# LowLevelAI/GLARE

Hardware: AMD Instinct MI355X
Metric: enhanced images/sec (400x600) (higher is better)
Workload: dtype fp16; 1 GPU; LOL eval15-shaped 400x600 inference, batch=8 per GPU, full encoder->flow->VQ->decoder->AFT (BASELINE configs[1]); batch_per_gpu=8, global_batch=8, input=3x400x600 (reflect-padded to 420x620), parallelism=dp1, streams_per_gpu=2, exchange=none (1 GPU), ranks_seen=1, weights=random, name-seeded (no checkpoints offline)

## Files before the change

glare_amd/csrc/conv_igemm.hip:

```cpp
#include "conv_igemm_kernel.h"

namespace {

__device__ __forceinline__ void pack_weight_chunk(const float* __restrict__ w, a16_t* __restrict__ out, long long chunk, int Cout, int Cin,
                                                  int KS, int TN, int KSTEPS, int n_stages, int dgrad, int Cin_real) {
  long long t = chunk;
  const int n = t % TN; t /= TN;
  const int khalf = t % 2; t /= 2;
  const int ks = t % KSTEPS; t /= KSTEPS;
  const int KK = KS * KS;
  const int tap = t % KK; t /= KK;
  const int s = t % n_stages; t /= n_stages;
  const int ct = (int)t;
  const int co = ct * TN + n;
  const int ci0 = (s * KSTEPS + ks) * 16 + khalf * 8;
  float v[8];
#pragma unroll
  for (int e = 0; e < 8; ++e) {
    const int ci = ci0 + e;
    v[e] = 0.f;
    if (dgrad) {
      if (co < Cout && ci < Cin_real) v[e] = w[((size_t)ci * Cout + co) * KK + (KK - 1 - tap)];
    } else if (co < Cout && ci < Cin) {
      v[e] = w[((size_t)co * Cin + ci) * KK + tap];
// ... 253 lines not shown
}

extern "C" int glare_conv2d_bf16(const glare_conv_desc* d, glare_stream_t stream_) {
  if (!d || !d->in || !d->weight_packed || !d->out) return GLARE_ERR_INVALID;
  if (d->B <= 0 || d->H <= 0 || d->W <= 0 || d->Cin <= 0 || d->Cout <= 0) return GLARE_ERR_INVALID;
  if (d->ksize != 1 && d->ksize != 3) return GLARE_ERR_UNSUPPORTED;
  if (d->stride != 1 && d->stride != 2) return GLARE_ERR_UNSUPPORTED;
  if (d->stride == 2 && (d->ksize != 3 || d->upsample)) return GLARE_ERR_UNSUPPORTED;
  const bool subpix = d->upsample == 2;
  if (subpix && (d->ksize != 3 || d->stride != 1)) return GLARE_ERR_UNSUPPORTED;
  if ((d->Cin % 8) || (d->in_pitch % 8) || (d->in_off % 8)) return GLARE_ERR_UNSUPPORTED;
  if (d->in2 && ((d->Cin2 % 8) || (d->in2_pitch % 8) || (d->in2_off % 8) || d->Cin2 <= 0)) return GLARE_ERR_UNSUPPORTED;
  if (d->out_mode < GLARE_OUT_NHWC_BF16 || d->out_mode > GLARE_OUT_PLANAR_BF16) return GLARE_ERR_INVALID;
  if (d->residual && d->out_mode > GLARE_OUT_NHWC_F32) return GLARE_ERR_UNSUPPORTED;
  if (d->in_off + d->Cin > d->in_pitch || d->out_off + d->Cout > d->out_pitch) return GLARE_ERR_INVALID;

  ConvParams p;
  p.in0 = (const a16_t*)d->in;
  p.in1 = (const a16_t*)d->in2;
  p.wpk = (const a16_t*)d->weight_packed;
  p.bias = d->bias;
  p.res = (const a16_t*)d->residual;
  p.out = d->out;
  p.B = d->B; p.H = d->H; p.W = d->W;
  p.IHs = (d->upsample && !subpix) ? 2 * d->H : d->H;
  p.IWs = (d->upsample && !subpix) ? 2 * d->W : d->W;
  if (d->stride == 2) {
    p.OH = (p.IHs + 1 - 3) / 2 + 1;
    p.OW = (p.IWs + 1 - 3) / 2 + 1;
  } else {
    p.OH = p.IHs; p.OW = p.IWs;
  }
  if (d->k_wrap < 0 || d->k_wrap > 2 || (d->k_wrap == 2 && !(d->in2 && d->Cin2 == d->Cin))) return GLARE_ERR_INVALID;
  if (d->k_wrap == 2 && (d->ksize != 3 || d->gn_coef || d->upsample || d->Cin % 16)) return GLARE_ERR_UNSUPPORTED;
  p.k_wrap = d->k_wrap;
  p.Cin0 = d->Cin; p.Cin1 = d->in2 ? d->Cin2 : 0; p.CinTot = p.Cin0 + p.Cin1 + (p.k_wrap ? p.Cin0 : 0);
  p.p0 = d->in_pitch; p.o0 = d->in_off; p.p1 = d->in2_pitch; p.o1 = d->in2_off;
  p.Cout = d->Cout; p.opitch = d->out_pitch; p.ooff = d->out_off;
  p.rpitch = d->res_pitch; p.roff = d->res_off;
  p.upsample = subpix ? 0 : d->upsample; p.act = d->act; p.out_mode = d->out_mode;
  p.plane_pitch = d->plane_pitch > 0 ? d->plane_pitch : (long long)p.OH * p.OW;
  if (p.plane_pitch < (long long)p.OH * p.OW) return GLARE_ERR_INVALID;
  if (d->cout_tile != 0 && (d->upsample == 2 || (d->cout_tile != 32 && d->cout_tile != 64 && d->cout_tile != 128))) return GLARE_ERR_INVALID;
  const Variant v = pick_variant(d->ksize, d->Cout, d->cout_tile);
  if (d->gn_partial && v.tn == 32 && d->Cout > 32) return GLARE_ERR_UNSUPPORTED;
  const int kc = 16 * v.ksteps;
  if ((p.in1 || p.k_wrap) && (p.Cin0 % kc)) return GLARE_ERR_UNSUPPORTED;
  if (p.k_wrap && (p.Cin1 % kc)) return GLARE_ERR_UNSUPPORTED;
  if (p.k_wrap && (subpix || d->upsample)) return GLARE_ERR_UNSUPPORTED;
  p.n_stages = (p.CinTot + kc - 1) / kc;
  {
    const long long b0 = (long long)p.H * p.W * p.p0 * 2, b1 = p.in1 ? (long long)p.H * p.W * p.p1 * 2 : 0;
    if (b0 >= 0x7ff00000LL || b1 >= 0x7ff00000LL) return GLARE_ERR_UNSUPPORTED;
    p.in0_bytes = (unsigned)b0;
    p.in1_bytes = (unsigned)b1;
    const long long br = d->residual ? (long long)p.OH * p.OW * p.rpitch * 2 : 0;
    p.res_bytes = (br > 0 && br < 0x7ff00000LL && !subpix) ? (unsigned)br : 0u;
    static const bool no_prefetch = getenv("GLARE_CONV_NO_RES_PREFETCH") != nullptr;
    if (no_prefetch) p.res_bytes = 0;
  }
  p.tiles_x = cdiv(p.OW, TW); p.tiles_y = 0; p.co_tiles = cdiv(p.Cout, v.tn);
  p.n_blocks = 0;
  p.gn_part = d->gn_partial;
  p.gn_nparts = 0;
  p.res_lo = (const a16_t*)d->residual_lo;
  p.out_lo = (a16_t*)d->out_lo;
  p.groups = d->groups > 1 ? d->groups : 1;
  p.g_in_step = d->group_in_step; p.g_out_step = d->group_out_step; p.g_bias_step = d->Cout; p.g_w_elems = 0;
  if (p.groups > 1) {
    if ((d->in2 && !(p.k_wrap && d->in2_pitch == d->in_pitch && d->Cin2 == d->Cin)) || d->residual || d->gn_partial || subpix || p.groups > 65535)
      return GLARE_ERR_UNSUPPORTED;
    if ((d->group_in_step % 8) || d->in_off + (long long)(p.groups - 1) * d->group_in_step + d->Cin > d->in_pitch ||
        d->out_off + (long long)(p.groups - 1) * d->group_out_step + d->Cout > d->out_pitch || d->group_out_step < 0 || d->group_in_step < 0)
      return GLARE_ERR_INVALID;
    p.g_w_elems = glare_conv2d_packed_weight_elems_tile(d->Cout, p.CinTot, d->ksize, d->cout_tile);
    if (d->in2 && d->in2_off + (long long)(p.groups - 1) * d->group_in_step + d->Cin2 > d->in2_pitch) return GLARE_ERR_INVALID;
  }
  p.gn_coef = d->gn_coef; p.gn_swish = d->gn_swish;
  if (p.gn_coef && (d->ksize != 3 || d->stride != 1 || d->in2 || p.k_wrap || d->upsample || p.groups > 1 || p.out_lo || d->in_off != 0 ||
                    d->Cin > 512))
    return GLARE_ERR_UNSUPPORTED;
  if (p.res_lo && !(p.res && p.out_lo)) return GLARE_ERR_INVALID;
  p.fast_epilogue = (d->out_mode == GLARE_OUT_NHWC_BF16) && !(p.Cout % 8) && !(p.opitch % 8) && !(p.ooff % 8) &&
                    (!p.res || (!(p.rpitch % 8) && !(p.roff % 8)));
  hipStream_t stream = (hipStream_t)stream_;

  if (p.out_lo) {
    if (subpix || d->upsample || !p.fast_epilogue) return GLARE_ERR_UNSUPPORTED;
    if (d->ksize == 1) return glare_conv_launch_k1(p, v.tn, true, stream);
    return d->stride == 2 ? glare_conv_launch_k3s2(p, v.tn, true, stream) : glare_conv_launch_k3s1(p, v.tn, true, stream);
  }
  if (subpix) {
    if (!p.fast_epilogue) return GLARE_ERR_UNSUPPORTED;
    return glare_conv_launch_k2(p, v.tn, stream);
  }
  if (d->ksize == 1) return glare_conv_launch_k1(p, v.tn, false, stream);
  if (d->stride == 2) return glare_conv_launch_k3s2(p, v.tn, false, stream);
  return glare_conv_launch_k3s1(p, v.tn, false, stream);
}

extern "C" long long glare_conv2d_gn_partial_elems(int B, int OH, int OW, int Cout) {
  if (B <= 0 || OH <= 0 || OW <= 0 || Cout <= 0) return GLARE_ERR_INVALID;
  const long long parts = (long long)cdiv(OW, TW) * cdiv(OH, 8) * 2;
  return (long long)B * parts * (Cout / 4) * 2;
}

extern "C" long long glare_conv2d_upsample_gn_partial_elems(int B, int H, int W, int Cout) {
  if (B <= 0 || H <= 0 || W <= 0 || Cout <= 0) return GLARE_ERR_INVALID;
  return 4 * glare_conv2d_gn_partial_elems(B, H, W, Cout);
}

extern "C" int glare_conv2d_upsample_gn_reduce(const float* gn_partial, float* stats_out, int B, int H, int W, int Cout,
                                               glare_stream_t stream) {
// ... 14 lines not shown
```

glare_amd/csrc/conv_igemm_k3s1.hip:

```cpp
#include "conv_igemm_kernel.h"

int glare_conv_launch_k3s1(const ConvParams& p, int tn, bool hilo, hipStream_t stream) {
  if (hilo) return tn == 128 ? launch<3, 1, 4, 2, 2, 2, 1, true>(p, stream) : GLARE_ERR_UNSUPPORTED;
  const int epi = conv_pick_epilogue(p, true);
  if (p.gn_coef) return (tn == 128 && epi == EPI_FAST) ? launch<3, 1, 4, 2, 2, 2, 1, false, true>(p, stream) : GLARE_ERR_UNSUPPORTED;
  if (epi == EPI_PLANAR) return glare_conv_launch_k3s1_planar(p, tn, stream);
  if (epi == EPI_GENERAL) return glare_conv_launch_k3s1_general(p, tn, stream);
  if (tn == 128) return launch<3, 1, 4, 2, 2, 2, 1>(p, stream);
  if (tn == 64) return launch<3, 1, 4, 1, 2, 2, 1>(p, stream);
  return launch<3, 1, 2, 1, 4, 1, 1>(p, stream);
}
```

glare_amd/csrc/conv_igemm_kernel.h:

```cpp
#pragma once
#include <type_traits>

#include "common.h"



struct ConvParams {
  const a16_t* in0;
  const a16_t* in1;
  const a16_t* wpk;
  const float* bias;
  const a16_t* res;
  void* out;
  int B, H, W;
  int IHs, IWs;
  int OH, OW;
  int Cin0, Cin1, CinTot;
  int p0, o0, p1, o1;
  int Cout, opitch, ooff, rpitch, roff;
  int upsample, act, out_mode;
  long long plane_pitch;
  int tiles_x, tiles_y, co_tiles, n_blocks, n_stages;
  int fast_epilogue;
  unsigned in0_bytes, in1_bytes;
  unsigned res_bytes;
  float* gn_part;
  int gn_nparts;
  const a16_t* res_lo;
  a16_t* out_lo;
  int groups, g_in_step, g_out_step, g_bias_step;
  long long g_w_elems;
  int k_wrap;
  const float* gn_coef;
  int gn_swish;
};

enum { EPI_FAST = 0,
       EPI_PLANAR = 1,
       EPI_GENERAL = 2 };
__host__ inline int conv_pick_epilogue(const ConvParams& p, bool planar_kernel) {
  const bool expk = p.act == GLARE_ACT_SIGMOID || p.act == GLARE_ACT_SWISH;
  if (p.out_mode == GLARE_OUT_NHWC_BF16 && p.fast_epilogue && !(p.res == nullptr && expk)) return EPI_FAST;
  if (planar_kernel && p.out_mode == GLARE_OUT_PLANAR_F32 && !p.res && !expk) return EPI_PLANAR;
  return EPI_GENERAL;
}

int glare_conv_launch_k3s1(const ConvParams& p, int tn, bool hilo, hipStream_t stream);
int glare_conv_launch_k3s1_planar(const ConvParams& p, int tn, hipStream_t stream);
int glare_conv_launch_k3s1_general(const ConvParams& p, int tn, hipStream_t stream);
int glare_conv_launch_k3s2(const ConvParams& p, int tn, bool hilo, hipStream_t stream);
int glare_conv_launch_k3s2_general(const ConvParams& p, int tn, hipStream_t stream);
int glare_conv_launch_k1(const ConvParams& p, int tn, bool hilo, hipStream_t stream);
int glare_conv_launch_k1_general(const ConvParams& p, int tn, hipStream_t stream);
int glare_conv_launch_k2(const ConvParams& p, int tn, hipStream_t stream);

namespace {

constexpr int TW = 32;



template <int KS, int STRIDE, int TH>
struct TileGeom {
  static constexpr int IH = (TH - 1) * STRIDE + KS;
  static constexpr int IW = (TW - 1) * STRIDE + KS;
  static constexpr int NPOS = IH * IW;
  static constexpr int PAD = (KS == 3 && STRIDE == 1) ? 1 : 0;
};

template <int N, typename F>
__device__ __forceinline__ void static_for(F&& f) {
  if constexpr (N > 0) {
    static_for<N - 1>(f);
    f(std::integral_constant<int, N - 1>{});
  }
}



__device__ __forceinline__ int fresh_lane_id() {
  int l;
  asm volatile("v_mbcnt_lo_u32_b32 %0, -1, 0\n\tv_mbcnt_hi_u32_b32 %0, -1, %0" : "=v"(l));
  return l;
}

__device__ __forceinline__ void gn_prologue_piece(u32x4* slot, const float* cf, int swish) {
  __builtin_amdgcn_sched_barrier(0);
  u32x4 v = *slot;
#pragma unroll
  for (int e = 0; e < 4; ++e) {
    const f32x4 q = *reinterpret_cast<const f32x4*>(cf + 4 * e);
    float lo = alo(v[e]) * q[0] + q[1];
    float hi = ahi(v[e]) * q[2] + q[3];
    if (swish) { lo = swishf_(lo); hi = swishf_(hi); }
    v[e] = pack_a2(lo, hi);
    __builtin_amdgcn_sched_barrier(0);
  }
  *slot = v;
  __builtin_amdgcn_sched_barrier(0);
}

template <int KS, int STRIDE, int MT, int NT, int WM, int WN, int KSTEPS, bool HILO = false, bool GNP = false, int EPI = EPI_FAST>
__global__ __launch_bounds__(64 * WM * WN, ((STRIDE == 1 && WM * WN == 4) ? 3 : 2)) void conv_igemm_kernel(const ConvParams p_in) {
  ConvParams p = p_in;
  if (p.groups > 1) {
    const int g = blockIdx.y;
    p.o0 += g * p.g_in_step;
    p.o1 += g * p.g_in_step;
    p.ooff += g * p.g_out_step;
    p.wpk += (size_t)g * p.g_w_elems;
    if (p.bias) p.bias += g * p.g_bias_step;
  }
  constexpr int TH = WM * MT;
  constexpr int NW = WM * WN;
  using G = TileGeom<KS, STRIDE, TH>;
  static_assert(NW == 4 || NW == 6 || NW == 8, "wave layout");
  constexpr int TN = WN * NT * 32;
  constexpr int A_CHUNKS = KSTEPS * 2 * G::NPOS;
  constexpr int A_INSTR = (A_CHUNKS + 63) / 64;
  constexpr int A_SLOTS = A_INSTR * 64;
  constexpr int A_PER_W = (A_INSTR + NW - 1) / NW;
  constexpr int B_CHUNKS = KS * KSTEPS * 2 * TN;
  static_assert(B_CHUNKS % 64 == 0, "B stage is a whole number of wave DMAs");
  constexpr int B_INSTR = B_CHUNKS / 64;
  constexpr int B_PER_W = (B_INSTR + NW - 1) / NW;
  constexpr int KC = 16 * KSTEPS;

  extern __shared__ __attribute__((aligned(16))) char smem[];
  u32x4* lA = reinterpret_cast<u32x4*>(smem);
  u32x4* lB = lA + 2 * A_SLOTS;

  int bid = blockIdx.x;
// ... 23 lines not shown
#pragma unroll
    for (int j = 0; j < NT; ++j)
#pragma unroll
      for (int r = 0; r < 16; ++r) acc[i][j][r] = 0.f;

  constexpr unsigned A_OOB = 0x80000000u;
  unsigned a_vo0[A_PER_W], a_vo1[A_PER_W];
  int a_ck[A_PER_W];
#pragma unroll
  for (int i = 0; i < A_PER_W; ++i) {
    const int c = (wave + NW * i) * 64 + lane;
    a_vo0[i] = a_vo1[i] = A_OOB;
    a_ck[i] = 0;
    if (c < A_CHUNKS) {
      const int prow = c / (2 * KSTEPS * G::IW), rem = c % (2 * KSTEPS * G::IW);
      const int kk = rem / G::IW, pos = prow * G::IW + rem % G::IW;
      a_ck[i] = kk * 8;
      const int iy = iy0 + pos / G::IW, ix = ix0 + pos % G::IW;
      if (iy >= 0 && iy < p.IHs && ix >= 0 && ix < p.IWs) {
        const int sy = p.upsample ? (iy >> 1) : iy, sx = p.upsample ? (ix >> 1) : ix;
        const unsigned pix = (unsigned)(sy * p.W + sx);
        a_vo0[i] = (pix * (unsigned)p.p0 + (unsigned)(p.o0 + kk * 8)) * 2u;
        if constexpr (!GNP) a_vo1[i] = (pix * (unsigned)p.p1 + (unsigned)(p.o1 + kk * 8)) * 2u;
      }
    }
  }
  const size_t img = (size_t)b * p.H * p.W;
  const __amdgpu_buffer_rsrc_t arsrc0 =
      __builtin_amdgcn_make_buffer_rsrc(const_cast<a16_t*>(p.in0 + img * p.p0), 0, (int)p.in0_bytes, 0x00020000);
  const __amdgpu_buffer_rsrc_t arsrc1 = __builtin_amdgcn_make_buffer_rsrc(
      const_cast<a16_t*>(p.in1 ? p.in1 + img * p.p1 : p.in0), 0, (int)(p.in1 ? p.in1_bytes : p.in0_bytes), 0x00020000);
  const a16_t* wbase = p.wpk + ((size_t)phase * p.co_tiles + ct) * p.n_stages * (size_t)(KS * B_CHUNKS) * 8;

  const bool reuse = KS == 3 && !GNP && p.k_wrap == 2;
  const int n_pair = reuse ? 2 * (p.Cin0 / KC) : 0;
  auto a_is_new = [&](int stage) { return !(reuse && stage < n_pair && (stage & 1)); };
  auto issue_a = [&](int chunk, int buf, int i_lo = 0, int i_hi = 1 << 20) {
    const int c0 = chunk * KC;
    bool src0 = GNP || c0 < p.Cin0 || c0 >= p.Cin0 + p.Cin1;
    int cbase = c0 < p.Cin0 ? c0 : (src0 ? c0 - p.Cin0 - p.Cin1 : c0 - p.Cin0);
    if (reuse) {
      src0 = chunk < n_pair;
      cbase = src0 ? (chunk >> 1) * KC : (chunk - n_pair) * KC;
    }
    const int climit = src0 ? p.Cin0 : p.Cin1;
#pragma unroll
    for (int i = 0; i < A_PER_W; ++i) {
      const int j = wave + NW * i;
      if (i >= i_lo && i < i_hi && j < A_INSTR) {
        unsigned vo = src0 ? a_vo0[i] : a_vo1[i];
        if (cbase + a_ck[i] >= climit) vo = A_OOB;
        if (src0)
          __builtin_amdgcn_raw_ptr_buffer_load_lds(arsrc0, (__attribute__((address_space(3))) void*)(lA + buf * A_SLOTS + j * 64), 16, vo,
                                                   cbase * 2, 0, 0);
        else
          __builtin_amdgcn_raw_ptr_buffer_load_lds(arsrc1, (__attribute__((address_space(3))) void*)(lA + buf * A_SLOTS + j * 64), 16, vo,
                                                   cbase * 2, 0, 0);
      }
    }
  };
  const __amdgpu_buffer_rsrc_t wrsrc = __builtin_amdgcn_make_buffer_rsrc(
      const_cast<a16_t*>(wbase), 0, (int)((size_t)p.n_stages * KS * B_CHUNKS * 16), 0x00020000);
  const int lane16 = lane * 16;
  auto issue_b = [&](int bstage, int buf, int i_lo = 0, int i_hi = 1 << 20) {
#pragma unroll
    for (int i = 0; i < B_PER_W; ++i) {
      const int j = wave + NW * i;
      if (i >= i_lo && i < i_hi && j < B_INSTR)
        __builtin_amdgcn_raw_ptr_buffer_load_lds(wrsrc, (__attribute__((address_space(3))) void*)(lB + buf * B_CHUNKS + j * 64),
                                                 16, lane16, (bstage * B_CHUNKS + j * 64) * 16, 0, 0);
    }
  };

  [[maybe_unused]] auto prefetch_residual = [&](int free_buf) {
    if constexpr (KS == 3 && STRIDE == 1 && NW == 4 && TN == 128) {
      static_assert(A_SLOTS * 16 >= NW * 4 * 256, "room for the prefetch's landing zone");
      const size_t rimg = (size_t)b * p.OH * p.OW * p.rpitch;
#pragma unroll
      for (int k = 0; k < 2; ++k) {
        const int l = (wave * 2 + k) * 64 + lane;
        const int oy = oy0 + (l >> 6), ox = ox0 + ((l >> 1) & 31), co = ct * TN + (l & 1) * 64;
        const unsigned vo = (oy < p.OH && ox < p.OW && co < p.Cout)
                                ? (unsigned)(((oy * p.OW + ox) * p.rpitch + p.roff + co) * 2) : 0x80000000u;
        const __amdgpu_buffer_rsrc_t rr = __builtin_amdgcn_make_buffer_rsrc(const_cast<a16_t*>(p.res + rimg), 0, (int)p.res_bytes, 0x00020000);
        __builtin_amdgcn_raw_ptr_buffer_load_lds(rr, (__attribute__((address_space(3))) void*)(lA + free_buf * A_SLOTS + (wave * 4 + k) * 16),
                                                 4, vo, 0, 0, 0);
        if constexpr (HILO) {
          if (p.res_lo) {
            const __amdgpu_buffer_rsrc_t rl =
                __builtin_amdgcn_make_buffer_rsrc(const_cast<a16_t*>(p.res_lo + rimg), 0, (int)p.res_bytes, 0x00020000);
            __builtin_amdgcn_raw_ptr_buffer_load_lds(rl, (__attribute__((address_space(3))) void*)(lA + free_buf * A_SLOTS + (wave * 4 + 2 + k) * 16),
                                                     4, vo, 0, 0, 0);
          }
        }
      }
    }
  };

  [[maybe_unused]] float* lC = reinterpret_cast<float*>(lB + 2 * B_CHUNKS);
  [[maybe_unused]] auto gn_transform = [&](int chunk, int buf) {
    if constexpr (GNP) {
      const int c0 = chunk * KC;
#pragma unroll
      for (int i = 0; i < A_PER_W; ++i) {
        const int j = wave + NW * i;
        if (j < A_INSTR && a_vo0[i] != A_OOB && c0 + a_ck[i] < p.Cin0) {
          int ln = fresh_lane_id(), ck = a_ck[i];
          asm volatile("" : "+v"(ln), "+v"(ck));
          gn_prologue_piece(lA + buf * A_SLOTS + j * 64 + ln, lC + (c0 + ck) * 2, p.gn_swish);
        }
      }
    }
  };
  if constexpr (GNP) {
    const float* src = p.gn_coef + (size_t)b * p.Cin0 * 2;
    for (int i = tid; i < p.Cin0 * 2; i += 64 * NW) lC[i] = src[i];
    __syncthreads();
  }

  const int khalf = lane >> 5, px = lane & 31;
  const int n_bstages = p.n_stages * KS;
  issue_a(0, 0);
  issue_b(0, 0);
  int bs = 0;
  int a_cnt = 0;
  for (int chunk = 0; chunk < p.n_stages; ++chunk) {
    const u32x4* cA = lA + (a_cnt & 1) * A_SLOTS;
    const bool next_new = chunk + 1 < p.n_stages && a_is_new(chunk + 1);
#pragma unroll
    for (int trow = 0; trow < KS; ++trow, ++bs) {
      asm volatile("s_waitcnt vmcnt(0)" ::: "memory");
      if constexpr (GNP) {
        if (trow == 0 && chunk == 0) gn_transform(0, 0);
        if (trow == 1 && chunk + 1 < p.n_stages) gn_transform(chunk + 1, (a_cnt + 1) & 1);
      }
      __syncthreads();
      constexpr int NGRP = KS * KSTEPS;
      [[maybe_unused]] constexpr int B_PG = (B_PER_W + NGRP - 1) / NGRP, A_PG = (A_PER_W + NGRP - 1) / NGRP;
      const bool more_b = bs + 1 < n_bstages, more_a = trow == 0 && next_new;
      if (trow == 0 && chunk + 1 == p.n_stages && p.res_bytes) prefetch_residual((a_cnt + 1) & 1);
      const u32x4* cB = lB + (bs & 1) * B_CHUNKS;
#pragma unroll
      for (int tcol = 0; tcol < KS; ++tcol) {
#pragma unroll
        for (int ks = 0; ks < KSTEPS; ++ks) {
          {
            const int grp = tcol * KSTEPS + ks;
            if (more_b) issue_b(bs + 1, (bs + 1) & 1, grp * B_PG, (grp + 1) * B_PG);
            if (more_a) issue_a(chunk + 1, (a_cnt + 1) & 1, grp * A_PG, (grp + 1) * A_PG);
          }
          a16x8 bf[NT], af[MT];
#pragma unroll
          for (int j = 0; j < NT; ++j) {
            const int co = (wn * NT + j) * 32 + px;
            bf[j] = __builtin_bit_cast(a16x8, cB[((tcol * KSTEPS + ks) * 2 + khalf) * TN + co]);
          }
#pragma unroll
          for (int i = 0; i < MT; ++i) {
            const int row = wm * MT + i;
            af[i] = __builtin_bit_cast(a16x8, cA[((row * STRIDE + trow) * (2 * KSTEPS) + ks * 2 + khalf) * G::IW + px * STRIDE + tcol]);
          }
#pragma unroll
          for (int i = 0; i < MT; ++i)
#pragma unroll
            for (int j = 0; j < NT; ++j)
              acc[i][j] = mfma_a16_32x32x16(af[i], bf[j], acc[i][j], 0, 0, 0);
        }
      }
    }
    if (next_new) ++a_cnt;
  }

  if constexpr (HILO) {
    constexpr int ROWF = NT * 128 + 16;
    constexpr int CPR = NT * 4;
    static_assert(NW * 32 * ROWF <= (2 * A_SLOTS + 2 * B_CHUNKS) * 16, "hi/lo epilogue slab fits the pipeline LDS");
    static_assert(KS != 2, "the sub-pixel form has no hi/lo epilogue");
    __syncthreads();
    char* slab = smem + wave * (32 * ROWF);
    const int lane = fresh_lane_id();
    const int ncol = lane & 31, rhalf = lane >> 5;
    float gs0 = 0.f, gq0 = 0.f, gs1 = 0.f, gq1 = 0.f;
// ... 287 lines not shown
        } else {
          if (co_ok && row_ok) {
            const size_t base = ((size_t)b * p.opitch + p.ooff + co) * (size_t)p.plane_pitch + (size_t)oy * p.OW + xb;
#pragma unroll
            for (int e = 0; e < 4; ++e) {
              if (xb + e < p.OW) {
                const float y = act_any(v[e], asel);
                if (p.out_mode == GLARE_OUT_PLANAR_F32)
                  reinterpret_cast<float*>(p.out)[base + e] = y;
                else
                  reinterpret_cast<a16_t*>(p.out)[base + e] = f2a(y);
              }
            }
          }
        }
      }
    });
  });
  }
}

template <int KS, int STRIDE, int MT, int NT, int WM, int WN, int KSTEPS, bool HILO = false, bool GNP = false, int EPI = EPI_FAST>
int launch(const ConvParams& p_in, hipStream_t stream) {
  using G = TileGeom<KS, STRIDE, WM * MT>;
  constexpr int TN = WN * NT * 32;
  ConvParams p = p_in;
  p.tiles_y = cdiv(p.OH, WM * MT);
  const long long nb = (long long)p.B * p.tiles_x * p.tiles_y * p.co_tiles * (KS == 2 ? 4 : 1);
  if (nb > 0x7fffffffLL) return GLARE_ERR_INVALID;
  p.n_blocks = (int)nb;
  p.gn_nparts = p.tiles_x * cdiv(p.OH, 8) * 2 * (KS == 2 ? 4 : 1);
  if (p.gn_part && !(p.fast_epilogue && p.Cout % 32 == 0)) return GLARE_ERR_UNSUPPORTED;
  if (p.gn_part && !HILO && EPI != EPI_FAST) return GLARE_ERR_UNSUPPORTED;
  const size_t lds = (size_t)(2 * (((KSTEPS * 2 * G::NPOS + 63) / 64) * 64) + 2 * KS * KSTEPS * 2 * TN) * 16 + (GNP ? (size_t)p.Cin0 * 8 : 0);
  constexpr bool PLANAR_KERNEL = !HILO && KS == 3 && STRIDE == 1 && WM * WN == 4;
  if (!HILO && conv_pick_epilogue(p, PLANAR_KERNEL) != EPI) return GLARE_ERR_INVALID;
  auto kern = conv_igemm_kernel<KS, STRIDE, MT, NT, WM, WN, KSTEPS, HILO, GNP, EPI>;
  if (lds > 64 * 1024 &&
      hipFuncSetAttribute((const void*)kern, hipFuncAttributeMaxDynamicSharedMemorySize, (int)lds) != hipSuccess)
    return GLARE_ERR_LAUNCH;
  hipLaunchKernelGGL(kern, dim3(p.n_blocks, p.groups > 1 ? p.groups : 1), dim3(64 * WM * WN), lds, stream, p);
  return glare_launch_status();
}

}
```

glare_amd/modules/encoder_decoder.py:

```python
import math
import os
import threading

import torch
import torch.nn as nn

from .. import autograd as A
from .. import ops
from ._base import HipModule, packed_conv, to_nchw, to_nhwc


GN_FUSED = True


def Normalize(in_channels):
    return nn.GroupNorm(num_groups=32, num_channels=in_channels, eps=1e-6, affine=True)


def gn_swish(x, norm, swish=True, pair=False):
    return ops.groupnorm(x, norm.weight.detach().float(), norm.bias.detach().float(), swish=swish, eps=norm.eps, pair=pair)


def is_hilo(x):
    return getattr(x, "_lo", None) is not None
# ... 4 lines not shown


def conv_t(x, conv, **kw):
    return A.conv2d(x, conv.weight, conv.bias, **kw)


HILO_STREAM = os.environ.get("GLARE_HILO_STREAM", "1") != "0"
FP32_CLASS = os.environ.get("GLARE_FP32_CLASS", "1") != "0"


_FP32_TLS = threading.local()


def fp32_class_on():
    v = getattr(_FP32_TLS, "value", None)
    return FP32_CLASS if v is None else v


class fp32_class:

    def __init__(self, on):
        self.on = bool(on)

    def __enter__(self):
        self._prev = getattr(_FP32_TLS, "value", None)
        _FP32_TLS.value = self.on
        return self

    def __exit__(self, *exc):
        _FP32_TLS.value = self._prev


GN_PROLOGUE = os.environ.get("GLARE_GN_PROLOGUE", "0") == "1"
SUBPIXEL_UPSAMPLE = True
FOLD_PROJ_INTO_V = True
SHARED_KV_ATTENTION = True
GN_FOLDED_ATTENTION = True


class Upsample(HipModule):
    def __init__(self, in_channels, with_conv=True):
        super().__init__()
        assert with_conv, "GLARE always resamples with a conv (resamp_with_conv=True)"
        self.with_conv = with_conv
        self.conv = nn.Conv2d(in_channels, in_channels, 3, 1, 1)

    def forward_nhwc(self, x, **kw):
        if SUBPIXEL_UPSAMPLE:
            pc = self._packed(("conv_subpixel", id(self.conv)),
                              lambda: ops.PackedConv(self.conv.weight, self.conv.bias, upsample_subpixel=True))
        else:
            pc = packed_conv(self, self.conv)
        return ops.conv2d(x, pc, upsample=True, gn_stats=GN_FUSED and self.conv.out_channels % 128 == 0, **kw)

    def train_nhwc(self, x):
        return conv_t(x, self.conv, upsample=True)

    def forward(self, x):
        return to_nchw(self.forward_nhwc(to_nhwc(x)))


class Downsample(HipModule):
    def __init__(self, in_channels, with_conv=True):
        super().__init__()
        assert with_conv
        self.with_conv = with_conv
        self.conv = nn.Conv2d(in_channels, in_channels, 3, 2, 0)

    def forward_nhwc(self, x, split=0):
        return ops.conv2d(x, packed_conv(self, self.conv, split=split), stride=2,
                          gn_stats=GN_FUSED and self.conv.out_channels % 128 == 0, hilo=is_hilo(x))

    def train_nhwc(self, x):
        return conv_t(x, self.conv, stride=2)

    def forward(self, x):
        return to_nchw(self.forward_nhwc(to_nhwc(x)))


class ResnetBlock(HipModule):
    def __init__(self, *, in_channels, out_channels=None, conv_shortcut=False, dropout=0.0, temb_channels=0):
        super().__init__()
        assert temb_channels == 0 and not conv_shortcut and dropout == 0.0
        out_channels = in_channels if out_channels is None else out_channels
        self.in_channels, self.out_channels = in_channels, out_channels
        self.norm1 = Normalize(in_channels)
        self.conv1 = nn.Conv2d(in_channels, out_channels, 3, 1, 1)
        self.norm2 = Normalize(out_channels)
        self.conv2 = nn.Conv2d(out_channels, out_channels, 3, 1, 1)
        if in_channels != out_channels:
            self.nin_shortcut = nn.Conv2d(in_channels, out_channels, 1, 1, 0)

    def forward_nhwc(self, x, out=None, out_off=0, split=0):
        fuse = GN_FUSED and self.out_channels % 128 == 0
        hl = is_hilo(x)
        if split:
            assert hl and out is None and split == 3
            h = ops.conv2d(gn_swish(x, self.norm1, pair=True), packed_conv(self, self.conv1, split=3), gn_stats=fuse, hilo=True)
            h = gn_swish(h, self.norm2, pair=True)
            res = x if self.in_channels == self.out_channels else ops.conv2d(x, packed_conv(self, self.nin_shortcut, split=3), hilo=True)
            return ops.conv2d(h, packed_conv(self, self.conv2, split=3), residual=res, gn_stats=fuse, hilo=True)
        if GN_PROLOGUE and not hl and self.in_channels <= 128 and getattr(x, "_gn_stats", None) is not None:
            coef = lambda t, n: ops.groupnorm_coeffs(t, n.weight.detach().float(), n.bias.detach().float(), n.eps)
            h = ops.conv2d(x, packed_conv(self, self.conv1), gn_stats=fuse, gn_prologue=(coef(x, self.norm1), True))
            if fuse and self.out_channels <= 128 and out is None:
                return ops.conv2d(h, packed_conv(self, self.conv2), gn_prologue=(coef(h, self.norm2), True),
                                  residual=x if self.in_channels == self.out_channels else ops.conv2d(x, packed_conv(self, self.nin_shortcut)),
                                  gn_stats=fuse)
        else:
            h = ops.conv2d(gn_swish(x, self.norm1), packed_conv(self, self.conv1), gn_stats=fuse)
        h = gn_swish(h, self.norm2)
        res = x if self.in_channels == self.out_channels else ops.conv2d(x, packed_conv(self, self.nin_shortcut), hilo=hl)
        return ops.conv2d(h, packed_conv(self, self.conv2), residual=res, out=out, out_off=out_off,
                          gn_stats=fuse and out is None, hilo=hl)

    def train_nhwc(self, x):
        x, xr = A.fork(x)
        h = conv_t(gn_swish_t(x, self.norm1), self.conv1)
        h = gn_swish_t(h, self.norm2)
        res = xr if self.in_channels == self.out_channels else conv_t(xr, self.nin_shortcut)
        return conv_t(h, self.conv2, residual=res)

    def forward(self, x, temb=None):
        return to_nchw(self.forward_nhwc(to_nhwc(x)))


class AttnBlock(HipModule):
    def __init__(self, in_channels):
        super().__init__()
        assert in_channels % 32 == 0, "AttnBlock: channels must be a multiple of 32 (GroupNorm(32), 32-wide GEMM k-steps)"
        self.in_channels = in_channels
        self.norm = Normalize(in_channels)
        self.q = nn.Conv2d(in_channels, in_channels, 1)
        self.k = nn.Conv2d(in_channels, in_channels, 1)
# ... 265 lines not shown
```

glare_amd/ops.py:

```python
import ctypes
import os

import torch

from . import _lib
from ._lib import act_dtype, check, host_f32, inference_precision, precision, ptr, require_cuda, stream_handle, use_precision


def vq_nearest(z_tokens, codebook, want_zq=True):
    require_cuda(z_tokens, codebook)
    assert z_tokens.dtype == torch.float32 and codebook.dtype == torch.float32
    z_tokens = z_tokens.contiguous()
    codebook = codebook.contiguous()
    n, dim = z_tokens.shape
    idx = torch.empty(n, dtype=torch.int64, device=z_tokens.device)
    zq = torch.empty_like(z_tokens) if want_zq else None
    check(_lib.lib().glare_vq_nearest_f32(ptr(z_tokens), ptr(codebook), n, codebook.shape[0], dim, ptr(idx), ptr(zq),
                                          stream_handle()), "glare_vq_nearest_f32")
    return idx, zq


_K = _lib.constants()
ACT = {name: _K["GLARE_ACT_" + name.upper()] for name in ("none", "relu", "sigmoid", "swish")}
OUT_NHWC_BF16, OUT_NHWC_F32, OUT_PLANAR_F32, OUT_PLANAR_BF16 = (_K["GLARE_OUT_" + n] for n in ("NHWC_BF16", "NHWC_F32", "PLANAR_F32", "PLANAR_BF16"))
# ... 424 lines not shown
def _ws_eligible(pc, x, cin, in_off, x2, stride, upsample, out_mode, out, out_off, residual, res_off, gn_stats, hilo, gn_prologue):
    if not (CONV1X1_WEIGHT_STATIONARY and x2 is None and stride == 1 and not upsample and out_mode == OUT_NHWC_BF16 and cin == pc.cin
            and x.shape[3] % 8 == 0 and in_off % 8 == 0
            and (out is None or (out.dtype == act_dtype() and out.shape[3] % 8 == 0 and out_off % 8 == 0))
            and (residual is None or (residual.shape[3] % 8 == 0 and res_off % 8 == 0))):
        return False
    whole = out is None or (out_off == 0 and out.shape[3] == pc.cout)
    if pc.split == 0:
        return pc.w16 is not None and (not gn_stats or out is None)
    if pc.split == 3:
        return (pc.ksize == 1 and pc.w16_lo is not None and gn_prologue is None and (not hilo or whole)
                and (not gn_stats or (pc.cout % 128 == 0 and whole)))
    return False


def conv2d(x, pc, *, x2=None, cin=None, in_off=0, cin2=None, in2_off=0, stride=1, upsample=False, act="none",
           residual=None, res_off=0, out=None, out_off=0, out_mode=OUT_NHWC_BF16, plane_pitch=0, gn_stats=False, hilo=False,
           gn_prologue=None):
    require_cuda(x, x2, residual, out)
    assert x.dtype == act_dtype() and x.dim() == 4 and x.is_contiguous(), (x.dtype, act_dtype())
    assert pc.packed.dtype == x.dtype, "filter packed under another precision"
    B, H, W, pitch = x.shape
    cin = pitch - in_off if cin is None else cin
    split = pc.split
    _count_conv_flops(pc, B * H * W * (4 if upsample else 1) // (stride * stride))
    if hilo and pc.ksize == 1 and not split:
        assert x2 is None and stride == 1 and not upsample and out is None and cin == pc.cin and pc.w16 is not None
        return _conv1x1_ws(x, pc, cin, in_off, act, residual, res_off, None, 0, gn_stats, True)
    if _ws_eligible(pc, x, cin, in_off, x2, stride, upsample, out_mode, out, out_off, residual, res_off, gn_stats, hilo, gn_prologue):
        return _conv1x1_ws(x, pc, cin, in_off, act, residual, res_off, out, out_off, gn_stats, hilo)
    cin2_total = 0
    if split:
        assert x2 is None and not upsample and cin == pc.cin, (cin, pc.cin)
        assert pc.k_wrap != 2 or gn_prologue is None
    elif x2 is not None:
        assert x2.dtype == act_dtype() and x2.is_contiguous() and x2.shape[:3] == x.shape[:3]
        cin2_total = x2.shape[3] - in2_off if cin2 is None else cin2
    assert pc.cin == cin + cin2_total, (pc.cin, cin, cin2_total)
    IH, IW = (2 * H, 2 * W) if upsample else (H, W)
    OH, OW = ((IH + 1 - 3) // 2 + 1, (IW + 1 - 3) // 2 + 1) if stride == 2 else (IH, IW)
    if out is None:
        if out_mode in (OUT_NHWC_BF16, OUT_NHWC_F32):
            out = torch.empty(B, OH, OW, pc.cout, dtype=act_dtype() if out_mode == OUT_NHWC_BF16 else torch.float32, device=x.device)
        else:
            pp = plane_pitch or OH * OW
            dt = torch.float32 if out_mode == OUT_PLANAR_F32 else act_dtype()
            out = torch.empty(B, pc.cout, pp, dtype=dt, device=x.device)
            if pp > OH * OW:
                out[:, :, OH * OW:].zero_()
    assert out.is_contiguous()
    if (AUTO_COUT_TILE and pc.ksize == 3 and pc.cout > 64 and pc.cout_tile == 0 and not pc.subpixel and pc._src is not None
            and not hilo and gn_prologue is None):
        tile = conv_cout_tile(B, OH, OW, pc.cout)
        if tile == 32 and gn_stats:
            tile = 64
        if tile:
            if tile not in pc._tiles:
                pc._tiles[tile] = PackedConv(pc._src[0], pc._src[1], dgrad_pad=pc._src[2], cout_tile=tile)
            pc = pc._tiles[tile]
    d = _conv_desc(x, pc, cin, in_off)
    if x2 is not None:
        d.in2, d.Cin2, d.in2_pitch, d.in2_off = x2.data_ptr(), cin2_total, x2.shape[3], in2_off
    if out_mode in (OUT_NHWC_BF16, OUT_NHWC_F32):
        d.out_pitch = out.shape[3]
    else:
        d.out_pitch, d.plane_pitch = out.shape[1], out.shape[2]
    d.out, d.out_off = out.data_ptr(), out_off
    if residual is not None:
        assert residual.dtype == act_dtype() and residual.is_contiguous()
        d.residual, d.res_pitch, d.res_off = residual.data_ptr(), residual.shape[3], res_off
    out_lo = None
    if hilo:
        assert out_mode == OUT_NHWC_BF16 and out_off == 0 and out.shape[3] == pc.cout
        out_lo = getattr(out, "_lo", None)
        if out_lo is None:
            out_lo = torch.empty_like(out)
        d.out_lo = out_lo.data_ptr()
        rlo = getattr(residual, "_lo", None) if residual is not None else None
        if rlo is not None:
            assert rlo.shape == residual.shape and rlo.dtype == residual.dtype and rlo.is_contiguous()
            d.residual_lo = rlo.data_ptr()
    if gn_prologue is not None:
        coef, swish = gn_prologue
        assert coef.dtype == torch.float32 and coef.is_contiguous() and tuple(coef.shape) == (B, cin, 2)
        assert pc.ksize == 3 and stride == 1 and x2 is None and not upsample and not split and not hilo and in_off == 0
        d.gn_coef, d.gn_swish = coef.data_ptr(), int(bool(swish))
    assert not pc.subpixel or upsample, "a sub-pixel packed filter only implements the upsample conv"
    d.stride, d.upsample, d.act, d.out_mode = stride, (2 if pc.subpixel else int(bool(upsample))), ACT[act], out_mode
    lib = _lib.lib()
    gn = None
    if gn_stats:
        assert out_mode == OUT_NHWC_BF16 and pc.cout % 128 == 0 and out_off == 0 and out.shape[3] == pc.cout
        gn = _GnStats("glare_conv2d_upsample", (B, H, W, pc.cout), x.device) if pc.subpixel else _GnStats("glare_conv2d", (B, OH, OW, pc.cout), x.device)
        d.gn_partial = gn.partial.data_ptr()
    if LAUNCH_EVENTS is not None and pc.ksize == 3:
        opix = B * OH * OW
        esz = 2 if out_mode in (OUT_NHWC_BF16, OUT_PLANAR_BF16) else 4
        with _timed_launch("conv3x3_split" if split else "conv3x3", 2.0 * opix * 9 * pc.cin * pc.cout,
                           2.0 * B * H * W * pc.cin * (2 if split == 3 else 1) + esz * opix * pc.cout * (2 if hilo else 1)
                           + 2.0 * 9 * pc.cin * pc.cout * (split or 1)):
            check(lib.glare_conv2d_bf16(ctypes.byref(d), stream_handle()), "glare_conv2d_bf16")
    else:
        check(lib.glare_conv2d_bf16(ctypes.byref(d), stream_handle()), "glare_conv2d_bf16")
    if gn is not None:
        gn.reduce(out)
    if out_lo is not None:
        out._lo = out_lo
    return out


def _workspace(nbytes, device):
    return torch.empty(max(int(nbytes), 16), dtype=torch.uint8, device=device)


def conv2d_smallcin(x, strides, shape_bhw, weight, bias=None, act="none", out=None, out_off=0, out_f32=False, hilo=False):
    require_cuda(x, weight, bias, out)
    B, H, W = shape_bhw
    w = weight.detach().float().contiguous()
# ... 476 lines not shown
```

Before: 63.57 images/sec.

## Fuse hi/lo pair GroupNorm+swish prologue into split-3 conv for 128-channel resblocks

Adds a GN-prologue variant of the hi/lo (split=3, k_wrap) 3x3 conv kernel. It loads both the hi and lo halves of each input tile, sums them, applies the GroupNorm affine plus swish in LDS, and re-splits into hi/lo before the MMA. This replaces the separate gn_swish pass that wrote a normalized pair tensor. It is enabled for 128-channel resblocks in split mode. The cost is extra LDS space for a companion buffer, additional loads, and more complex scheduling inside the main loop.

```diff
diff --git a/glare_amd/csrc/conv_igemm.hip b/glare_amd/csrc/conv_igemm.hip
--- a/glare_amd/csrc/conv_igemm.hip
+++ b/glare_amd/csrc/conv_igemm.hip
@@ -309,7 +309,7 @@
     p.OH = p.IHs; p.OW = p.IWs;
   }
   if (d->k_wrap < 0 || d->k_wrap > 2 || (d->k_wrap == 2 && !(d->in2 && d->Cin2 == d->Cin))) return GLARE_ERR_INVALID;
-  if (d->k_wrap == 2 && (d->ksize != 3 || d->gn_coef || d->upsample || d->Cin % 16)) return GLARE_ERR_UNSUPPORTED;
+  if (d->k_wrap == 2 && (d->ksize != 3 || d->upsample || d->Cin % 16)) return GLARE_ERR_UNSUPPORTED;
   p.k_wrap = d->k_wrap;
   p.Cin0 = d->Cin; p.Cin1 = d->in2 ? d->Cin2 : 0; p.CinTot = p.Cin0 + p.Cin1 + (p.k_wrap ? p.Cin0 : 0);
   p.p0 = d->in_pitch; p.o0 = d->in_off; p.p1 = d->in2_pitch; p.o1 = d->in2_off;
@@ -354,8 +354,10 @@
     if (d->in2 && d->in2_off + (long long)(p.groups - 1) * d->group_in_step + d->Cin2 > d->in2_pitch) return GLARE_ERR_INVALID;
   }
   p.gn_coef = d->gn_coef; p.gn_swish = d->gn_swish;
-  if (p.gn_coef && (d->ksize != 3 || d->stride != 1 || d->in2 || p.k_wrap || d->upsample || p.groups > 1 || p.out_lo || d->in_off != 0 ||
-                    d->Cin > 512))
+  if (p.gn_coef && (d->ksize != 3 || d->stride != 1 || d->upsample || p.groups > 1 || d->in_off != 0 || d->Cin > 512))
+    return GLARE_ERR_UNSUPPORTED;
+  if (p.gn_coef && (p.k_wrap || d->in2 || p.out_lo) &&
+      !(p.k_wrap && d->in2 && p.out_lo && d->Cin2 == d->Cin && d->in2_pitch == d->in_pitch && d->in2_off == 0 && d->Cin % 16 == 0))
     return GLARE_ERR_UNSUPPORTED;
   if (p.res_lo && !(p.res && p.out_lo)) return GLARE_ERR_INVALID;
   p.fast_epilogue = (d->out_mode == GLARE_OUT_NHWC_BF16) && !(p.Cout % 8) && !(p.opitch % 8) && !(p.ooff % 8) &&
diff --git a/glare_amd/csrc/conv_igemm_k3s1.hip b/glare_amd/csrc/conv_igemm_k3s1.hip
--- a/glare_amd/csrc/conv_igemm_k3s1.hip
+++ b/glare_amd/csrc/conv_igemm_k3s1.hip
@@ -1,6 +1,7 @@
 #include "conv_igemm_kernel.h"
 
 int glare_conv_launch_k3s1(const ConvParams& p, int tn, bool hilo, hipStream_t stream) {
+  if (hilo && p.gn_coef) return glare_conv_launch_k3s1_gnpair(p, tn, stream);
   if (hilo) return tn == 128 ? launch<3, 1, 4, 2, 2, 2, 1, true>(p, stream) : GLARE_ERR_UNSUPPORTED;
   const int epi = conv_pick_epilogue(p, true);
   if (p.gn_coef) return (tn == 128 && epi == EPI_FAST) ? launch<3, 1, 4, 2, 2, 2, 1, false, true>(p, stream) : GLARE_ERR_UNSUPPORTED;
diff --git a/glare_amd/csrc/conv_igemm_k3s1_gnpair.hip b/glare_amd/csrc/conv_igemm_k3s1_gnpair.hip
--- /dev/null
+++ b/glare_amd/csrc/conv_igemm_k3s1_gnpair.hip
@@ -0,0 +1,6 @@
+#include "conv_igemm_kernel.h"
+
+int glare_conv_launch_k3s1_gnpair(const ConvParams& p, int tn, hipStream_t stream) {
+  if (tn != 128 || !p.gn_coef || !p.k_wrap || !p.in1 || !p.out_lo) return GLARE_ERR_UNSUPPORTED;
+  return launch<3, 1, 4, 2, 2, 2, 1, true, true>(p, stream);
+}
diff --git a/glare_amd/csrc/conv_igemm_kernel.h b/glare_amd/csrc/conv_igemm_kernel.h
--- a/glare_amd/csrc/conv_igemm_kernel.h
+++ b/glare_amd/csrc/conv_igemm_kernel.h
@@ -46,6 +46,7 @@
 }
 
 int glare_conv_launch_k3s1(const ConvParams& p, int tn, bool hilo, hipStream_t stream);
+int glare_conv_launch_k3s1_gnpair(const ConvParams& p, int tn, hipStream_t stream);
 int glare_conv_launch_k3s1_planar(const ConvParams& p, int tn, hipStream_t stream);
 int glare_conv_launch_k3s1_general(const ConvParams& p, int tn, hipStream_t stream);
 int glare_conv_launch_k3s2(const ConvParams& p, int tn, bool hilo, hipStream_t stream);
@@ -98,6 +99,43 @@
   }
   *slot = v;
   __builtin_amdgcn_sched_barrier(0);
+}
+
+__device__ __forceinline__ void gn_prologue_piece_pair(u32x4* slot, const u32x4* other, const float* cf, int swish, bool want_lo) {
+  __builtin_amdgcn_sched_barrier(0);
+  u32x4 v = *slot;
+  const u32x4 w = *other;
+#pragma unroll
+  for (int h = 0; h < 2; ++h) {
+    const f32x4 q0 = *reinterpret_cast<const f32x4*>(cf + 8 * h), q1 = *reinterpret_cast<const f32x4*>(cf + 8 * h + 4);
+#pragma unroll
+    for (int k = 0; k < 2; ++k) {
+      const int e = 2 * h + k;
+      const f32x4 q = k ? q1 : q0;
+      float lo = (alo(v[e]) + alo(w[e])) * q[0] + q[1];
+      float hi = (ahi(v[e]) + ahi(w[e])) * q[2] + q[3];
+      if (swish) { lo = swishf_(lo); hi = swishf_(hi); }
+      uint32_t o = pack_a2(lo, hi);
+      if (want_lo) o = pack_a2(lo - alo(o), hi - ahi(o));
+      v[e] = o;
+    }
+    __builtin_amdgcn_sched_barrier(0);
+  }
+  *slot = v;
+  __builtin_amdgcn_sched_barrier(0);
+}
+
+__device__ __forceinline__ bool pair_stage_source(int chunk, int k_wrap, int two_n, int& chunk_out) {
+  const int r = chunk - two_n;
+  bool src0;
+  if (k_wrap == 2) {
+    src0 = r < 0;
+    chunk_out = r < 0 ? (chunk >> 1) : r;
+  } else {
+    src0 = r >= 0 || 2 * chunk < two_n;
+    chunk_out = r >= 0 ? r : (2 * chunk < two_n ? chunk : chunk - (two_n >> 1));
+  }
+  return __builtin_amdgcn_readfirstlane((int)src0) != 0;
 }
 
 template <int KS, int STRIDE, int MT, int NT, int WM, int WN, int KSTEPS, bool HILO = false, bool GNP = false, int EPI = EPI_FAST>
@@ -187,10 +225,11 @@
       const_cast<a16_t*>(p.in1 ? p.in1 + img * p.p1 : p.in0), 0, (int)(p.in1 ? p.in1_bytes : p.in0_bytes), 0x00020000);
   const a16_t* wbase = p.wpk + ((size_t)phase * p.co_tiles + ct) * p.n_stages * (size_t)(KS * B_CHUNKS) * 8;
 
-  const bool reuse = KS == 3 && !GNP && p.k_wrap == 2;
+  constexpr bool GNPAIR = GNP && HILO;
+  const bool reuse = KS == 3 && (!GNP || GNPAIR) && p.k_wrap == 2;
   const int n_pair = reuse ? 2 * (p.Cin0 / KC) : 0;
   auto a_is_new = [&](int stage) { return !(reuse && stage < n_pair && (stage & 1)); };
-  auto issue_a = [&](int chunk, int buf, int i_lo = 0, int i_hi = 1 << 20) {
+  auto issue_a = [&](int chunk, int buf, int i_lo = 0, int i_hi = 1 << 20, int comp = -1, int comp_step = 0) {
     const int c0 = chunk * KC;
     bool src0 = GNP || c0 < p.Cin0 || c0 >= p.Cin0 + p.Cin1;
     int cbase = c0 < p.Cin0 ? c0 : (src0 ? c0 - p.Cin0 - p.Cin1 : c0 - p.Cin0);
@@ -198,19 +237,24 @@
       src0 = chunk < n_pair;
       cbase = src0 ? (chunk >> 1) * KC : (chunk - n_pair) * KC;
     }
+    if constexpr (GNPAIR) {
+      src0 = pair_stage_source(chunk, p.k_wrap, 2 * (p.Cin0 / KC), cbase) != (comp >= 0);
+      cbase *= KC;
+    }
     const int climit = src0 ? p.Cin0 : p.Cin1;
 #pragma unroll
     for (int i = 0; i < A_PER_W; ++i) {
       const int j = wave + NW * i;
       if (i >= i_lo && i < i_hi && j < A_INSTR) {
-        unsigned vo = src0 ? a_vo0[i] : a_vo1[i];
-        if (cbase + a_ck[i] >= climit) vo = A_OOB;
+        unsigned vo = (GNP || src0) ? a_vo0[i] : a_vo1[i];
+        if constexpr (!GNPAIR) {
+          if (cbase + a_ck[i] >= climit) vo = A_OOB;
+        }
+        const int dst = (GNPAIR && comp >= 0) ? comp + j * comp_step : buf * A_SLOTS + j * 64;
         if (src0)
-          __builtin_amdgcn_raw_ptr_buffer_load_lds(arsrc0, (__attribute__((address_space(3))) void*)(lA + buf * A_SLOTS + j * 64), 16, vo,
-                                                   cbase * 2, 0, 0);
+          __builtin_amdgcn_raw_ptr_buffer_load_lds(arsrc0, (__attribute__((address_space(3))) void*)(lA + dst), 16, vo, cbase * 2, 0, 0);
         else
-          __builtin_amdgcn_raw_ptr_buffer_load_lds(arsrc1, (__attribute__((address_space(3))) void*)(lA + buf * A_SLOTS + j * 64), 16, vo,
-                                                   cbase * 2, 0, 0);
+          __builtin_amdgcn_raw_ptr_buffer_load_lds(arsrc1, (__attribute__((address_space(3))) void*)(lA + dst), 16, vo, cbase * 2, 0, 0);
       }
     }
   };
@@ -252,9 +296,27 @@
     }
   };
 
-  [[maybe_unused]] float* lC = reinterpret_cast<float*>(lB + 2 * B_CHUNKS);
+  [[maybe_unused]] constexpr int X_ROW = 2 * A_SLOTS + 2 * B_CHUNKS, X_FIRST = 2 * A_SLOTS + B_CHUNKS;
+  [[maybe_unused]] float* lC = reinterpret_cast<float*>(lB + 2 * B_CHUNKS + (GNPAIR ? NW * 64 : 0));
+  [[maybe_unused]] auto gn_transform_pair = [&](int chunk, int buf, int piece, int row, bool first = false) {
+    if constexpr (GNPAIR) {
+      int cbase;
+      const bool src0 = pair_stage_source(chunk, p.k_wrap, 2 * (p.Cin0 / KC), cbase);
+      cbase *= KC;
+#pragma unroll
+      for (int i = 0; i < A_PER_W; ++i) {
+        const int j = wave + NW * i;
+        if ((first || i == piece) && j < A_INSTR && a_vo0[i] != A_OOB) {
+          int ln = fresh_lane_id();
+          asm volatile("" : "+v"(ln));
+          const int ck = ((j * 64 + ln) % (2 * KSTEPS * G::IW)) / G::IW * 8;
+          gn_prologue_piece_pair(lA + buf * A_SLOTS + j * 64 + ln, lA + (first ? row + j * 64 : row) + ln, lC + (cbase + ck) * 2, p.gn_swish, !src0);
+        }
+      }
+    }
+  };
   [[maybe_unused]] auto gn_transform = [&](int chunk, int buf) {
-    if constexpr (GNP) {
+    if constexpr (GNP && !GNPAIR) {
       const int c0 = chunk * KC;
 #pragma unroll
       for (int i = 0; i < A_PER_W; ++i) {
@@ -276,6 +338,10 @@
   const int khalf = lane >> 5, px = lane & 31;
   const int n_bstages = p.n_stages * KS;
   issue_a(0, 0);
+  if constexpr (GNPAIR) {
+    static_assert(!GNPAIR || (KS == 3 && A_PER_W <= KS && A_SLOTS <= B_CHUNKS), "one companion piece per tap row; the first tile's fit a weight buffer");
+    issue_a(0, 0, 0, 1 << 20, X_FIRST, 64);
+  }
   issue_b(0, 0);
   int bs = 0;
   int a_cnt = 0;
@@ -285,11 +351,17 @@
 #pragma unroll
     for (int trow = 0; trow < KS; ++trow, ++bs) {
       asm volatile("s_waitcnt vmcnt(0)" ::: "memory");
-      if constexpr (GNP) {
+      if constexpr (GNPAIR) {
+        if (trow == 0 && chunk == 0) gn_transform_pair(0, 0, 0, X_FIRST, true);
+        if (trow == 0 && chunk > 0 && a_is_new(chunk)) gn_transform_pair(chunk, a_cnt & 1, KS - 1, X_ROW + wave * 64);
+      } else if constexpr (GNP) {
         if (trow == 0 && chunk == 0) gn_transform(0, 0);
         if (trow == 1 && chunk + 1 < p.n_stages) gn_transform(chunk + 1, (a_cnt + 1) & 1);
       }
       __syncthreads();
+      if constexpr (GNPAIR) {
+        if (trow >= 1 && next_new) gn_transform_pair(chunk + 1, (a_cnt + 1) & 1, trow - 1, X_ROW + wave * 64);
+      }
       constexpr int NGRP = KS * KSTEPS;
       [[maybe_unused]] constexpr int B_PG = (B_PER_W + NGRP - 1) / NGRP, A_PG = (A_PER_W + NGRP - 1) / NGRP;
       const bool more_b = bs + 1 < n_bstages, more_a = trow == 0 && next_new;
@@ -303,6 +375,9 @@
             const int grp = tcol * KSTEPS + ks;
             if (more_b) issue_b(bs + 1, (bs + 1) & 1, grp * B_PG, (grp + 1) * B_PG);
             if (more_a) issue_a(chunk + 1, (a_cnt + 1) & 1, grp * A_PG, (grp + 1) * A_PG);
+            if constexpr (GNPAIR) {
+              if (grp == 1 && next_new) issue_a(chunk + 1, 0, trow, trow + 1, X_ROW + wave * 64);
+            }
           }
           a16x8 bf[NT], af[MT];
 #pragma unroll
@@ -656,7 +731,8 @@
   p.gn_nparts = p.tiles_x * cdiv(p.OH, 8) * 2 * (KS == 2 ? 4 : 1);
   if (p.gn_part && !(p.fast_epilogue && p.Cout % 32 == 0)) return GLARE_ERR_UNSUPPORTED;
   if (p.gn_part && !HILO && EPI != EPI_FAST) return GLARE_ERR_UNSUPPORTED;
-  const size_t lds = (size_t)(2 * (((KSTEPS * 2 * G::NPOS + 63) / 64) * 64) + 2 * KS * KSTEPS * 2 * TN) * 16 + (GNP ? (size_t)p.Cin0 * 8 : 0);
+  const size_t lds = (size_t)(2 * (((KSTEPS * 2 * G::NPOS + 63) / 64) * 64) + 2 * KS * KSTEPS * 2 * TN) * 16 + (GNP ? (size_t)p.Cin0 * 8 : 0) +
+                     (GNP && HILO ? (size_t)WM * WN * 64 * 16 : 0);
   constexpr bool PLANAR_KERNEL = !HILO && KS == 3 && STRIDE == 1 && WM * WN == 4;
   if (!HILO && conv_pick_epilogue(p, PLANAR_KERNEL) != EPI) return GLARE_ERR_INVALID;
   auto kern = conv_igemm_kernel<KS, STRIDE, MT, NT, WM, WN, KSTEPS, HILO, GNP, EPI>;
diff --git a/glare_amd/modules/encoder_decoder.py b/glare_amd/modules/encoder_decoder.py
--- a/glare_amd/modules/encoder_decoder.py
+++ b/glare_amd/modules/encoder_decoder.py
@@ -60,6 +60,7 @@
 
 
 GN_PROLOGUE = os.environ.get("GLARE_GN_PROLOGUE", "0") == "1"
+PAIR_GN_PROLOGUE = {128: True, 256: False, 512: False}
 SUBPIXEL_UPSAMPLE = True
 FOLD_PROJ_INTO_V = True
 SHARED_KV_ATTENTION = True
@@ -124,10 +125,17 @@
         hl = is_hilo(x)
         if split:
             assert hl and out is None and split == 3
-            h = ops.conv2d(gn_swish(x, self.norm1, pair=True), packed_conv(self, self.conv1, split=3), gn_stats=fuse, hilo=True)
-            h = gn_swish(h, self.norm2, pair=True)
+
+            def normed_conv(t, norm, conv, **kw):
+                pc = packed_conv(self, conv, split=3)
+                if PAIR_GN_PROLOGUE.get(pc.cin, False) and pc.cin % 16 == 0 and getattr(t, "_gn_stats", None) is not None:
+                    coef = ops.groupnorm_coeffs(t, norm.weight.detach().float(), norm.bias.detach().float(), norm.eps)
+                    return ops.conv2d(t, pc, gn_prologue=(coef, True), gn_stats=fuse, hilo=True, **kw)
+                return ops.conv2d(gn_swish(t, norm, pair=True), pc, gn_stats=fuse, hilo=True, **kw)
+
+            h = normed_conv(x, self.norm1, self.conv1)
             res = x if self.in_channels == self.out_channels else ops.conv2d(x, packed_conv(self, self.nin_shortcut, split=3), hilo=True)
-            return ops.conv2d(h, packed_conv(self, self.conv2, split=3), residual=res, gn_stats=fuse, hilo=True)
+            return normed_conv(h, self.norm2, self.conv2, residual=res)
         if GN_PROLOGUE and not hl and self.in_channels <= 128 and getattr(x, "_gn_stats", None) is not None:
             coef = lambda t, n: ops.groupnorm_coeffs(t, n.weight.detach().float(), n.bias.detach().float(), n.eps)
             h = ops.conv2d(x, packed_conv(self, self.conv1), gn_stats=fuse, gn_prologue=(coef(x, self.norm1), True))
diff --git a/glare_amd/ops.py b/glare_amd/ops.py
--- a/glare_amd/ops.py
+++ b/glare_amd/ops.py
@@ -480,7 +480,6 @@
     cin2_total = 0
     if split:
         assert x2 is None and not upsample and cin == pc.cin, (cin, pc.cin)
-        assert pc.k_wrap != 2 or gn_prologue is None
     elif x2 is not None:
         assert x2.dtype == act_dtype() and x2.is_contiguous() and x2.shape[:3] == x.shape[:3]
         cin2_total = x2.shape[3] - in2_off if cin2 is None else cin2
@@ -531,7 +530,8 @@
     if gn_prologue is not None:
         coef, swish = gn_prologue
         assert coef.dtype == torch.float32 and coef.is_contiguous() and tuple(coef.shape) == (B, cin, 2)
-        assert pc.ksize == 3 and stride == 1 and x2 is None and not upsample and not split and not hilo and in_off == 0
+        assert pc.ksize == 3 and stride == 1 and x2 is None and not upsample and in_off == 0
+        assert (not split and not hilo) or (split == 3 and hilo and cin % 16 == 0), (split, hilo, cin)
         d.gn_coef, d.gn_swish = coef.data_ptr(), int(bool(swish))
     assert not pc.subpixel or upsample, "a sub-pixel packed filter only implements the upsample conv"
     d.stride, d.upsample, d.act, d.out_mode = stride, (2 if pc.subpixel else int(bool(upsample))), ACT[act], out_mode
```

Result: no change. 63.03 images/sec (-0.8%).
